# yisol/IDM-VTON

Measured on NVIDIA H100. Metric: try-on images/sec @768x1024, 30 steps, CFG 2.0, higher is better.
Workload: dtype fp16

## Files before the change

### idm-vton_b200/csrc/gemm.cu

```cuda
#include "gemm_common.cuh"
#include "host.h"
#include "wgmma.cuh"

namespace vton {

enum : int { KIND_F16 = 0, KIND_F16IN_F32OUT = 1, KIND_TF32 = 2, KIND_E4M3 = 3 };

constexpr bool f16_out(int kind) { return kind == KIND_F16 || kind == KIND_E4M3; }

template <int BN, int STAGES, bool GEGLU, int KIND>
struct SmemLayout {
  static constexpr int B_BYTES = BN * 128;
  static constexpr int STAGE_BYTES = A_BYTES + B_BYTES;
  static constexpr int STAGING_OFFSET = STAGES * STAGE_BYTES;
  static constexpr int STAGING_BYTES = f16_out(KIND) ? StagingTile<BN, GEGLU>::BYTES : 0;
  static constexpr int BAR_OFFSET = STAGING_OFFSET + STAGING_BYTES;
  static constexpr int ROWS_OFFSET = BAR_OFFSET + 256;
  static constexpr int TOTAL = ROWS_OFFSET + (f16_out(KIND) ? 2 * BM * 4 : 0) + 1024;
};

constexpr int GEMM_THREADS = 384;
constexpr int GEMM_PRODUCER_REGS = 56;
constexpr int GEMM_CONSUMER_REGS = 224;

template <int BN>
constexpr int E4M3_SUB = BN == 256 ? 64 : (BN == 192 ? 96 : BN);

template <int BN, int STAGES, bool GEGLU, bool SC, int KIND>
__global__ void __launch_bounds__(GEMM_THREADS, 1)
gemm_conv_kernel(const __grid_constant__ CUtensorMap tmA, const __grid_constant__ CUtensorMap tmB,
                 const __grid_constant__ CUtensorMap tmS0, const __grid_constant__ CUtensorMap tmS1,
                 const __grid_constant__ CUtensorMap tmBs, const GemmParams p) {
  using L = SmemLayout<BN, STAGES, GEGLU, KIND>;
  constexpr int KBK = KIND == KIND_TF32 ? 32 : (KIND == KIND_E4M3 ? 128 : 64);
  constexpr bool F16_EPI = f16_out(KIND);
  extern __shared__ uint8_t smem_raw[];
  const uint32_t smem_base = (smem_u32(smem_raw) + 1023u) & ~1023u;
  const uint32_t bar_base = smem_base + L::BAR_OFFSET;
  auto full_bar = [&](int s) { return bar_base + 8u * s; };
  auto empty_bar = [&](int s) { return bar_base + 8u * (STAGES + s); };
  const uint32_t staged_bar = bar_base + 8u * (2 * STAGES);
  const uint32_t ready_bar = bar_base + 8u * (2 * STAGES + 1);
  const uint32_t staging = smem_base + L::STAGING_OFFSET;
  auto staging_ptr = [&]() { return smem_raw + (smem_base - smem_u32(smem_raw)) + L::STAGING_OFFSET; };
  auto row_table = [&]() { return reinterpret_cast<int*>(smem_raw + (smem_base - smem_u32(smem_raw)) + L::ROWS_OFFSET); };

  const int warp = threadIdx.x >> 5;

  if (threadIdx.x == 8 * 32) {
    tma_prefetch_desc(&tmA);
    tma_prefetch_desc(&tmB);
    if (SC) {
      tma_prefetch_desc(&tmS0);
      tma_prefetch_desc(&tmS1);
      tma_prefetch_desc(&tmBs);
    }
    for (int s = 0; s < STAGES; ++s) {
      mbar_init(full_bar(s), 1);
      mbar_init(empty_bar(s), 2);
    }
    if (F16_EPI) {
      mbar_init(staged_bar, 256);
      mbar_init(ready_bar, EpilogueStore<BN, GEGLU>::THREADS);
    }
    fence_barrier_init();
  }
  pdl_wait();
  __syncthreads();
  pdl_launch_dependents();

  if (warp >= 8) {
    setmaxnreg_dec<GEMM_PRODUCER_REGS>();
    if (threadIdx.x == 8 * 32) {
      const int total_slabs = p.slabs_main + (SC ? p.slabs_sc : 0);
      uint32_t it = 0;
      for (int tile = blockIdx.x; tile < p.total_tiles; tile += gridDim.x) {
        const int n0 = (tile % p.n_tiles) * BN;
        const int m_tile = tile / p.n_tiles;
        int b0 = 0, y0 = 0, x0 = 0;
        if (p.conv) {
          x0 = (m_tile % p.tiles_x) * p.bw;
          y0 = ((m_tile / p.tiles_x) % p.tiles_y) * p.bh;
          b0 = (m_tile / (p.tiles_x * p.tiles_y)) * p.bb;
        }
        for (int s = 0; s < total_slabs; ++s, ++it) {
          const int stage = it % STAGES;
          const uint32_t phase = (it / STAGES) & 1;
          mbar_wait(empty_bar(stage), phase ^ 1);
          const uint32_t a_dst = smem_base + stage * L::STAGE_BYTES;
          const uint32_t b_dst = a_dst + A_BYTES;
          mbar_expect_tx(full_bar(stage), L::STAGE_BYTES);
          if (s < p.slabs_main) {
            if (p.conv) {
              const int tap = s / p.cin_slabs;
              const int c0 = (s - tap * p.cin_slabs) * KBK;
              const int dy = tap / 3 - 1, dx = tap % 3 - 1;
              tma_load_4d(a_dst, &tmA, full_bar(stage), c0, x0 * p.stride + dx, y0 * p.stride + dy, b0);
              tma_load_2d(b_dst, &tmB, full_bar(stage), c0, tap * p.cout + n0);
            } else {
              tma_load_2d(a_dst, &tmA, full_bar(stage), s * KBK, m_tile * BM);
              tma_load_2d(b_dst, &tmB, full_bar(stage), s * KBK, n0);
            }
          } else {
            const int ss = s - p.slabs_main;
            if (ss < p.sc_split)
              tma_load_4d(a_dst, &tmS0, full_bar(stage), ss * BK, x0, y0, b0);
            else
              tma_load_4d(a_dst, &tmS1, full_bar(stage), (ss - p.sc_split) * BK, x0, y0, b0);
            tma_load_2d(b_dst, &tmBs, full_bar(stage), ss * BK, n0);
          }
        }
      }
    } else if (F16_EPI && warp > 8) {
      EpilogueStore<BN, GEGLU>::run(p, staging, staging_ptr(), row_table(), staged_bar, ready_bar, threadIdx.x - 9 * 32);
    }
    return;
  }

  setmaxnreg_inc<GEMM_CONSUMER_REGS>();
  const int wg = warp >> 2;
  const int lane = threadIdx.x & 31;
  const int r_local = wg * 64 + ((warp & 3) << 4) + (lane >> 2);
  float acc[BN / 2];
  float acc_sc[BN / 2];
  uint32_t it = 0;
  auto release = [&](uint32_t slab) {
    if ((threadIdx.x & 127) == 0) mbar_arrive(empty_bar(slab % STAGES));
  };
  auto run_slabs = [&](float (&accr)[BN / 2], int s_begin, int s_end) {
    for (int s = s_begin; s < s_end; ++s, ++it) {
      const int stage = it % STAGES;
      mbar_wait(full_bar(stage), (it / STAGES) & 1);
      const uint32_t a_src = smem_base + stage * L::STAGE_BYTES + wg * (64 * 128);
      const uint32_t b_src = smem_base + stage * L::STAGE_BYTES + A_BYTES;
      wgmma_fence();
#pragma unroll
      for (int k = 0; k < 4; ++k) {
        const uint64_t da = make_gmma_desc_sw128(a_src + k * 32, 0, 1024);
        const uint64_t db = make_gmma_desc_sw128(b_src + k * 32, 0, 1024);
        const int scale_d = (s > s_begin || k > 0) ? 1 : 0;
        if constexpr (KIND == KIND_TF32) {
          WgmmaTF32SS<BN>::mma(accr, da, db, scale_d);
        } else {
          WgmmaF16SS<BN, 0>::mma(accr, da, db, scale_d);
        }
      }
      wgmma_commit();
      wgmma_wait<1>();
      if (s > 0) release(it - 1);
    }
  };
  auto run_slabs_promoted = [&](float (&accr)[BN / 2], int s_begin, int s_end) {
    constexpr int SUB = E4M3_SUB<BN>;
    for (int s = s_begin; s < s_end; ++s, ++it) {
      const int stage = it % STAGES;
      mbar_wait(full_bar(stage), (it / STAGES) & 1);
      const uint32_t a_src = smem_base + stage * L::STAGE_BYTES + wg * (64 * 128);
      const uint32_t b_src = smem_base + stage * L::STAGE_BYTES + A_BYTES;
#pragma unroll
      for (int sub = 0; sub < BN / SUB; ++sub) {
        float part[SUB / 2];
        wgmma_fence();
#pragma unroll
        for (int k = 0; k < 4; ++k) {
          const uint64_t da = make_gmma_desc_sw128(a_src + k * 32, 0, 1024);
          const uint64_t db = make_gmma_desc_sw128(b_src + sub * SUB * 128 + k * 32, 0, 1024);
          WgmmaE4M3SS<SUB>::mma(part, da, db, k > 0 ? 1 : 0);
        }
        wgmma_commit();
        wgmma_wait<0>();
        fence_regs(part);
#pragma unroll
        for (int j = 0; j < SUB / 2; ++j) accr[sub * (SUB / 2) + j] = s > s_begin ? accr[sub * (SUB / 2) + j] + part[j] : part[j];
      }
      release(it);
    }
  };
  for (int tile = blockIdx.x; tile < p.total_tiles; tile += gridDim.x) {
    EpilogueF16<BN, GEGLU, SC, KIND == KIND_E4M3> epi;
    if constexpr (F16_EPI) epi.begin(p, tile / p.n_tiles, tile % p.n_tiles, r_local);
    if constexpr (KIND == KIND_E4M3) {
      run_slabs_promoted(acc, 0, p.slabs_main);
    } else {
      run_slabs(acc, 0, p.slabs_main);
      if constexpr (SC) run_slabs(acc_sc, p.slabs_main, p.slabs_main + p.slabs_sc);
      wgmma_wait<0>();
      fence_regs(acc);
      if (SC) fence_regs(acc_sc);
      release(it - 1);
    }
    if constexpr (F16_EPI) {
      mbar_wait(ready_bar, ((tile - blockIdx.x) / gridDim.x) & 1);
      if (!GEGLU && p.act_gelu) epi.template stage<true, true>(p, acc, acc_sc, r_local, staging);
      else if (!GEGLU && p.rowvec) epi.template stage<false, true>(p, acc, acc_sc, r_local, staging);
      else epi.template stage<false, false>(p, acc, acc_sc, r_local, staging);
      mbar_arrive(staged_bar);
      if (tile + static_cast<int>(gridDim.x) >= p.total_tiles)
        EpilogueStore<BN, GEGLU>::help_store_last(p, tile, staging_ptr(), row_table(), staged_bar, threadIdx.x);
    } else {
      epilogue_f32<BN>(p, tile / p.n_tiles, tile % p.n_tiles, r_local, acc);
    }
  }
}

template <int BN, int STAGES, bool GEGLU, bool SC, int KIND>
static int launch_variant(const CUtensorMap& tmA, const CUtensorMap& tmB, const CUtensorMap& tmS0,
                          const CUtensorMap& tmS1, const CUtensorMap& tmBs, const GemmParams& p, cudaStream_t stream) {
  using L = SmemLayout<BN, STAGES, GEGLU, KIND>;
  static_assert(L::TOTAL <= 227 * 1024, "shared memory budget");
  auto kern = gemm_conv_kernel<BN, STAGES, GEGLU, SC, KIND>;
  static bool configured = false;
  if (!configured) {
    VTON_CUDA(cudaFuncSetAttribute(kern, cudaFuncAttributeMaxDynamicSharedMemorySize, L::TOTAL));
    configured = true;
  }
  const int grid = p.total_tiles < num_sms() ? p.total_tiles : num_sms();
  VTON_CUDA(launch_kernel(kern, dim3(grid), dim3(GEMM_THREADS), L::TOTAL, stream, tmA, tmB, tmS0, tmS1, tmBs, p));
  count_launch();
  return kOk;
}

void set_auto_v2(int) {}
void set_cluster4(int) {}

static int pick_bn(int N, int m_tiles, bool geglu, bool has_shortcut, int force_bn) {
  if (force_bn >= 2000) force_bn -= 2000;
  else if (force_bn >= 1000) force_bn -= 1000;
  auto usable = [&](int bn) {
    if (geglu && ((bn != 256 && bn != 128) || N % bn != 0)) return false;
    if (has_shortcut && bn > 128) return false;
    return true;
  };
  if (force_bn) {
    const bool known = force_bn == 64 || force_bn == 128 || force_bn == 160 || force_bn == 192 || force_bn == 256;
    return known && usable(force_bn) ? force_bn : 0;
  }
  const int sms = num_sms();
  const int cands[5] = {256, 192, 160, 128, 64};
  double best = 1e300;
  int best_bn = 0;
  for (int bn : cands) {
    if (!usable(bn)) continue;
    if (bn != 128 && N % bn != 0 && !(bn == 64 && N < 64)) continue;
    const long long tiles = static_cast<long long>(m_tiles) * cdiv(N, bn);
    const long long waves = (tiles + sms - 1) / sms;
    const double cost = static_cast<double>(waves) * (bn + 64);
    if (cost < best * 0.999) {
      best = cost;
      best_bn = bn;
    }
  }
  return best_bn ? best_bn : 128;
}

template <int KIND>
static int dispatch(int bn, bool geglu, const CUtensorMap& tmA, const CUtensorMap& tmB, const CUtensorMap& tmS0,
                    const CUtensorMap& tmS1, const CUtensorMap& tmBs, GemmParams& p, int m_tiles,
                    cudaStream_t stream) {
  p.n_tiles = cdiv(p.N, bn);
  p.total_tiles = m_tiles * p.n_tiles;
  if (geglu) {
    if (bn == 128) return launch_variant<128, 6, true, false, KIND>(tmA, tmB, tmS0, tmS1, tmBs, p, stream);
    if (bn == 256) return launch_variant<256, 4, true, false, KIND>(tmA, tmB, tmS0, tmS1, tmBs, p, stream);
    set_last_error("GEGLU epilogue supports BN 128/256 only (got %d)", bn);
    return kErrUnsupported;
  }
  if constexpr (KIND == KIND_F16) {
    if (p.slabs_sc) {
      if (bn == 64) return launch_variant<64, 8, false, true, KIND_F16>(tmA, tmB, tmS0, tmS1, tmBs, p, stream);
      if (bn == 128) return launch_variant<128, 6, false, true, KIND_F16>(tmA, tmB, tmS0, tmS1, tmBs, p, stream);
      set_last_error("shortcut epilogue supports BN 64/128 only (got %d)", bn);
      return kErrUnsupported;
    }
  }
  switch (bn) {
    case 64: return launch_variant<64, 8, false, false, KIND>(tmA, tmB, tmS0, tmS1, tmBs, p, stream);
    case 128: return launch_variant<128, 6, false, false, KIND>(tmA, tmB, tmS0, tmS1, tmBs, p, stream);
    case 160: return launch_variant<160, 5, false, false, KIND>(tmA, tmB, tmS0, tmS1, tmBs, p, stream);
    case 192: return launch_variant<192, 4, false, false, KIND>(tmA, tmB, tmS0, tmS1, tmBs, p, stream);
    case 256: return launch_variant<256, 3, false, false, KIND>(tmA, tmB, tmS0, tmS1, tmBs, p, stream);
  }
  set_last_error("unsupported BN %d", bn);
  return kErrUnsupported;
}

int gemm_f16_impl(const void* A, long long lda, const void* W, long long ldw, void* out, long long ldo, int M, int N,
                  int K, const void* bias, const void* residual, long long ldr, const void* rowvec, long long ld_rowvec,
                  int rows_per_sample, int flags, int force_bn, cudaStream_t stream) {
  const int geglu = flags & 1;
  VTON_CHECK_ARG(M > 0 && N > 0 && K > 0, "gemm: empty problem M=%d N=%d K=%d", M, N, K);
  VTON_CHECK_ARG(K % 64 == 0, "gemm: K=%d must be a multiple of 64", K);
  VTON_CHECK_ARG(N % 8 == 0 && lda % 8 == 0 && ldw % 8 == 0 && ldo % 8 == 0, "gemm: N/lda/ldw/ldo must be multiples of 8");
  VTON_CHECK_ARG(!geglu || (N % 16 == 0 && !residual && !rowvec), "gemm: bad GEGLU configuration");
  VTON_CHECK_ARG(aligned_to(out, 16) && aligned_to(bias, 16) && aligned_to(residual, 16) && aligned_to(rowvec, 16),
                 "gemm: out/bias/residual/rowvec must be 16-byte aligned");
  VTON_CHECK_ARG((!residual || ldr % 8 == 0) && (!rowvec || ld_rowvec % 8 == 0),
                 "gemm: ldr=%lld / ld_rowvec=%lld must be multiples of 8", ldr, ld_rowvec);
  const int bn = pick_bn(N, cdiv(M, BM), geglu != 0, false, force_bn);
  VTON_CHECK_ARG(bn != 0, "gemm: tile width force_bn=%d unsupported for this problem (N=%d, geglu=%d)", force_bn, N, geglu);
  VTON_CHECK_ARG(!geglu || N % bn == 0, "gemm: GEGLU needs N %% BN == 0 (N=%d, BN=%d)", N, bn);
  CUtensorMap tmA, tmB;
  {
    uint64_t dims[2] = {static_cast<uint64_t>(K), static_cast<uint64_t>(M)};
    uint64_t strides[1] = {static_cast<uint64_t>(lda) * 2};
    uint32_t box[2] = {64, 128};
    if (int e = encode_tmap_f16(&tmA, A, 2, dims, strides, box)) return e;
  }
  {
    uint64_t dims[2] = {static_cast<uint64_t>(K), static_cast<uint64_t>(N)};
    uint64_t strides[1] = {static_cast<uint64_t>(ldw) * 2};
    uint32_t box[2] = {64, static_cast<uint32_t>(bn)};
    if (int e = encode_tmap_f16(&tmB, W, 2, dims, strides, box)) return e;
  }
  GemmParams p{};
  p.out = static_cast<__half*>(out);
  p.ld_out = static_cast<int>(ldo);
  p.M = M;
  p.N = N;
  p.bias = static_cast<const __half*>(bias);
  p.residual = static_cast<const __half*>(residual);
  p.ld_res = static_cast<int>(ldr);
  p.rowvec = static_cast<const __half*>(rowvec);
  p.ld_rowvec = static_cast<int>(ld_rowvec);
  p.rows_per_sample = rows_per_sample;
  p.slabs_main = K / 64;
  p.act_gelu = (flags & 4) ? 2 : ((flags & 2) ? 1 : 0);
  return dispatch<KIND_F16>(bn, geglu != 0, tmA, tmB, tmA, tmA, tmB, p, cdiv(M, BM), stream);
}

int gemm_e4m3_impl(const void* A, long long lda, const void* a_scale, const void* W, long long ldw, const void* w_scale,
                   void* out, long long ldo, int M, int N, int K, const void* bias, const void* residual, long long ldr,
                   int flags, int force_bn, cudaStream_t stream) {
  const int geglu = flags & 1;
  VTON_CHECK_ARG(M > 0 && N > 0 && K > 0, "gemm_e4m3: empty problem M=%d N=%d K=%d", M, N, K);
  VTON_CHECK_ARG(K % 128 == 0, "gemm_e4m3: K=%d must be a multiple of 128", K);
  VTON_CHECK_ARG((flags & ~1) == 0, "gemm_e4m3: flags=%d unsupported (only GEGLU = 1)", flags);
  VTON_CHECK_ARG(A && W && out && a_scale && w_scale, "gemm_e4m3: A, W, out, a_scale and w_scale must not be null");
  VTON_CHECK_ARG(lda % 16 == 0 && ldw % 16 == 0, "gemm_e4m3: lda=%lld / ldw=%lld must be multiples of 16 bytes", lda, ldw);
  VTON_CHECK_ARG(N % 8 == 0 && ldo % 8 == 0, "gemm_e4m3: N/ldo must be multiples of 8");
  VTON_CHECK_ARG(!geglu || (N % 16 == 0 && !residual), "gemm_e4m3: bad GEGLU configuration");
  VTON_CHECK_ARG(aligned_to(A, 16) && aligned_to(W, 16) && aligned_to(out, 16) && aligned_to(bias, 16) &&
                     aligned_to(residual, 16) && aligned_to(a_scale, 4) && aligned_to(w_scale, 8),
                 "gemm_e4m3: A/W/out/bias/residual must be 16-byte aligned, a_scale 4-byte, w_scale 8-byte");
  VTON_CHECK_ARG(!residual || ldr % 8 == 0, "gemm_e4m3: ldr=%lld must be a multiple of 8", ldr);
  const int bn = pick_bn(N, cdiv(M, BM), geglu != 0, false, force_bn);
  VTON_CHECK_ARG(bn != 0, "gemm_e4m3: tile width force_bn=%d unsupported for this problem (N=%d, geglu=%d)", force_bn, N,
                 geglu);
  VTON_CHECK_ARG(!geglu || N % bn == 0, "gemm_e4m3: GEGLU needs N %% BN == 0 (N=%d, BN=%d)", N, bn);
  CUtensorMap tmA, tmB;
  {
    uint64_t dims[2] = {static_cast<uint64_t>(K), static_cast<uint64_t>(M)};
    uint64_t strides[1] = {static_cast<uint64_t>(lda)};
    uint32_t box[2] = {128, 128};
    if (int e = encode_tmap_u8(&tmA, A, 2, dims, strides, box)) return e;
  }
  {
    uint64_t dims[2] = {static_cast<uint64_t>(K), static_cast<uint64_t>(N)};
    uint64_t strides[1] = {static_cast<uint64_t>(ldw)};
    uint32_t box[2] = {128, static_cast<uint32_t>(bn)};
    if (int e = encode_tmap_u8(&tmB, W, 2, dims, strides, box)) return e;
  }
  GemmParams p{};
  p.out = static_cast<__half*>(out);
  p.ld_out = static_cast<int>(ldo);
  p.M = M;
  p.N = N;
  p.bias = static_cast<const __half*>(bias);
  p.residual = static_cast<const __half*>(residual);
  p.ld_res = static_cast<int>(ldr);
  p.slabs_main = K / 128;
  p.a_scale = static_cast<const float*>(a_scale);
  p.w_scale = static_cast<const float*>(w_scale);
  return dispatch<KIND_E4M3>(bn, geglu != 0, tmA, tmB, tmA, tmA, tmB, p, cdiv(M, BM), stream);
}

static void pick_box(int B, int H, int W, int* bw, int* bh, int* bb) {
  int w = 1;
  while (w < 128 && W % (w * 2) == 0) w *= 2;
  int h = 1;
  while (w * h < 128 && h * 2 <= H) h *= 2;
  *bw = w;
  *bh = h;
  *bb = 128 / (w * h);
  (void)B;
}

static int encode_nhwc(CUtensorMap* tm, const void* base, int B, int H, int W, int C, int ldc, int bw, int bh, int bb,
                       int pixel_step = 1) {
  uint64_t dims[4] = {static_cast<uint64_t>(C), static_cast<uint64_t>(W), static_cast<uint64_t>(H),
                      static_cast<uint64_t>(B)};
  uint64_t strides[3] = {static_cast<uint64_t>(ldc) * 2, static_cast<uint64_t>(W) * ldc * 2,
                         static_cast<uint64_t>(H) * W * ldc * 2};
  uint32_t box[4] = {64, static_cast<uint32_t>(bw * pixel_step), static_cast<uint32_t>(bh * pixel_step),
                     static_cast<uint32_t>(bb)};
  uint32_t estr[4] = {1, static_cast<uint32_t>(pixel_step), static_cast<uint32_t>(pixel_step), 1};
  return encode_tmap_f16(tm, base, 4, dims, strides, box, pixel_step > 1 ? estr : nullptr);
}

int conv3x3_impl(const void* x, long long ldx, int B, int Hin, int Win, int Cin, const void* w, int Cout, const void* bias,
                 const void* temb, long long ld_temb, const void* sc0, int C0, const void* sc1, int C1, const void* w_sc,
                 const void* bias_sc, const void* residual, long long ldr, void* out, long long ldo, int force_bn,
                 int stride, cudaStream_t stream) {
  VTON_CHECK_ARG(B > 0 && Hin > 0 && Win > 0, "conv3x3: empty input");
  VTON_CHECK_ARG(stride == 1 || stride == 2, "conv3x3: stride %d unsupported", stride);
  VTON_CHECK_ARG(stride == 1 || (!w_sc && !residual), "conv3x3: stride 2 has no shortcut / residual form");
  const int H = (Hin - 1) / stride + 1, W = (Win - 1) / stride + 1;
  VTON_CHECK_ARG(Cin % 64 == 0, "conv3x3: Cin=%d must be a multiple of 64 (pad channels)", Cin);
  VTON_CHECK_ARG(Cout % 8 == 0 && ldo % 8 == 0 && ldx % 8 == 0, "conv3x3: Cout/ldo/ldx must be multiples of 8");
  VTON_CHECK_ARG(C0 % 64 == 0 && C1 % 64 == 0, "conv3x3: shortcut source channels must be multiples of 64");
  VTON_CHECK_ARG(!(w_sc && residual), "conv3x3: shortcut conv and identity residual are exclusive");
  VTON_CHECK_ARG(aligned_to(out, 16) && aligned_to(bias, 16) && aligned_to(temb, 16) && aligned_to(bias_sc, 16) &&
                     aligned_to(residual, 16),
                 "conv3x3: out/bias/temb/bias_sc/residual must be 16-byte aligned");
  VTON_CHECK_ARG((!residual || ldr % 8 == 0) && (!temb || ld_temb % 8 == 0),
                 "conv3x3: ldr=%lld / ld_temb=%lld must be multiples of 8", ldr, ld_temb);
  int bw, bh, bb;
  pick_box(B, H, W, &bw, &bh, &bb);
  const int m_tiles_est = (W / bw) * cdiv(H, bh) * cdiv(B, bb);
  const int bn = pick_bn(Cout, m_tiles_est, false, w_sc != nullptr, force_bn);
  VTON_CHECK_ARG(bn != 0, "conv3x3: tile width force_bn=%d unsupported (a fused shortcut takes 64 or 128)", force_bn);
  CUtensorMap tmA, tmB, tmS0, tmS1, tmBs;
  VTON_CHECK_ARG(stride == 1 || (bw * 2 <= 256 && bh * 2 <= 256), "conv3x3: stride-2 box too large");
  if (int e = encode_nhwc(&tmA, x, B, Hin, Win, Cin, static_cast<int>(ldx), bw, bh, bb, stride)) return e;
  {
    uint64_t dims[2] = {static_cast<uint64_t>(Cin), static_cast<uint64_t>(9) * Cout};
    uint64_t strides[1] = {static_cast<uint64_t>(Cin) * 2};
    uint32_t box[2] = {64, static_cast<uint32_t>(bn)};
    if (int e = encode_tmap_f16(&tmB, w, 2, dims, strides, box)) return e;
  }
  tmS0 = tmA;
  tmS1 = tmA;
  tmBs = tmB;
  GemmParams p{};
  if (w_sc) {
    VTON_CHECK_ARG(sc0 && C0 > 0, "conv3x3: shortcut needs a source");
    if (int e = encode_nhwc(&tmS0, sc0, B, H, W, C0, C0, bw, bh, bb)) return e;
    if (sc1 && C1 > 0) {
      if (int e = encode_nhwc(&tmS1, sc1, B, H, W, C1, C1, bw, bh, bb)) return e;
    }
    const int Csc = C0 + (sc1 ? C1 : 0);
    uint64_t dims[2] = {static_cast<uint64_t>(Csc), static_cast<uint64_t>(Cout)};
    uint64_t strides[1] = {static_cast<uint64_t>(Csc) * 2};
    uint32_t box[2] = {64, static_cast<uint32_t>(bn)};
    if (int e = encode_tmap_f16(&tmBs, w_sc, 2, dims, strides, box)) return e;
    p.slabs_sc = Csc / 64;
    p.sc_split = C0 / 64;
  }
  p.out = static_cast<__half*>(out);
  p.ld_out = static_cast<int>(ldo);
  p.M = B * H * W;
  p.N = Cout;
  p.bias = static_cast<const __half*>(bias);
  p.bias_sc = static_cast<const __half*>(bias_sc);
  p.residual = static_cast<const __half*>(residual);
  p.ld_res = static_cast<int>(ldr);
  p.rowvec = static_cast<const __half*>(temb);
  p.ld_rowvec = static_cast<int>(ld_temb);
  p.slabs_main = 9 * (Cin / 64);
  p.conv = 1;
  p.stride = stride;
  p.H = H;
  p.W = W;
  p.B = B;
  p.bw = bw;
  p.bh = bh;
  p.bb = bb;
  p.tiles_x = W / bw;
  p.tiles_y = cdiv(H, bh);
  p.cin_slabs = Cin / 64;
  p.cout = Cout;
  const int m_tiles = p.tiles_x * p.tiles_y * cdiv(B, bb);
  return dispatch<KIND_F16>(bn, false, tmA, tmB, tmS0, tmS1, tmBs, p, m_tiles, stream);
}

int conv3x3_f32_impl(const void* x, int B, int H, int W, int Cin, const void* w, int Cout, const void* bias,
                     const void* residual, void* out, int in_fp16, cudaStream_t stream) {
  VTON_CHECK_ARG(B > 0 && H > 0 && W > 0, "conv3x3_f32: empty input");
  VTON_CHECK_ARG(Cin % 32 == 0 && Cout % 32 == 0 && Cout >= 64, "conv3x3_f32: Cin=%d / Cout=%d must be multiples of 32 (Cout >= 64)", Cin, Cout);
  VTON_CHECK_ARG(!in_fp16 || Cin % 64 == 0, "conv3x3_f32: fp16 operands need Cin=%d to be a multiple of 64", Cin);
  VTON_CHECK_ARG(x && w && out, "conv3x3_f32: null pointer");
  const int esz = in_fp16 ? 2 : 4;
  const int bk = in_fp16 ? 64 : 32;
  int bw, bh, bb;
  pick_box(B, H, W, &bw, &bh, &bb);
  VTON_CHECK_ARG(bw * bh * bb == 128 && bw >= 8, "conv3x3_f32: W=%d H=%d cannot be tiled into 128-pixel boxes", W, H);
  const int m_tiles = (W / bw) * cdiv(H, bh) * cdiv(B, bb);
  const int bn = pick_bn(Cout, m_tiles, false, false, Cout % 256 == 0 ? 256 : 128);
  CUtensorMap tmA, tmB;
  {
    uint64_t dims[4] = {static_cast<uint64_t>(Cin), static_cast<uint64_t>(W), static_cast<uint64_t>(H), static_cast<uint64_t>(B)};
    uint64_t strides[3] = {static_cast<uint64_t>(Cin) * esz, static_cast<uint64_t>(W) * Cin * esz,
                           static_cast<uint64_t>(H) * W * Cin * esz};
    uint32_t box[4] = {static_cast<uint32_t>(bk), static_cast<uint32_t>(bw), static_cast<uint32_t>(bh), static_cast<uint32_t>(bb)};
    if (int e = in_fp16 ? encode_tmap_f16(&tmA, x, 4, dims, strides, box) : encode_tmap_f32(&tmA, x, 4, dims, strides, box)) return e;
  }
  {
    uint64_t dims[2] = {static_cast<uint64_t>(Cin), static_cast<uint64_t>(9) * Cout};
    uint64_t strides[1] = {static_cast<uint64_t>(Cin) * esz};
    uint32_t box[2] = {static_cast<uint32_t>(bk), static_cast<uint32_t>(bn)};
    if (int e = in_fp16 ? encode_tmap_f16(&tmB, w, 2, dims, strides, box) : encode_tmap_f32(&tmB, w, 2, dims, strides, box)) return e;
  }
  GemmParams p{};
  p.out_f32 = static_cast<float*>(out);
  p.bias_f32 = static_cast<const float*>(bias);
  p.res_f32 = static_cast<const float*>(residual);
  p.M = B * H * W;
  p.N = Cout;
  p.slabs_main = 9 * (Cin / bk);
  p.conv = 1;
  p.stride = 1;
  p.H = H;
  p.W = W;
  p.B = B;
  p.bw = bw;
  p.bh = bh;
  p.bb = bb;
  p.tiles_x = W / bw;
  p.tiles_y = cdiv(H, bh);
  p.cin_slabs = Cin / bk;
  p.cout = Cout;
  p.n_tiles = cdiv(Cout, bn);
  p.total_tiles = m_tiles * p.n_tiles;
  if (in_fp16) {
    if (bn == 256) return launch_variant<256, 4, false, false, KIND_F16IN_F32OUT>(tmA, tmB, tmA, tmA, tmB, p, stream);
    return launch_variant<128, 6, false, false, KIND_F16IN_F32OUT>(tmA, tmB, tmA, tmA, tmB, p, stream);
  }
  if (bn == 256) return launch_variant<256, 4, false, false, KIND_TF32>(tmA, tmB, tmA, tmA, tmB, p, stream);
  return launch_variant<128, 6, false, false, KIND_TF32>(tmA, tmB, tmA, tmA, tmB, p, stream);
}

}
```

### idm-vton_b200/csrc/gemm_common.cuh

```cuda
#pragma once
#include "common.cuh"

namespace vton {

struct GemmParams {
  __half* out;
  int ld_out;
  int M, N;
  const __half* bias;
  const __half* bias_sc;
  const __half* residual;
  int ld_res;
  const __half* rowvec;
  int ld_rowvec;
  int rows_per_sample;
  int slabs_main;
  int slabs_sc;
  int sc_split;
  int conv;
  int H, W, B;
  int bw, bh, bb;
  int tiles_x, tiles_y;
  int cin_slabs;
  int cout;
  int n_tiles;
  int total_tiles;
  int act_gelu;
  int stride;
  float* out_f32;
  const float* bias_f32;
  const float* res_f32;
  const float* a_scale;
  const float* w_scale;
};

constexpr int BM = 128;
constexpr int BK = 64;
constexpr int A_BYTES = BM * BK * 2;

__device__ __forceinline__ void map_row(const GemmParams& p, int m_tile, int r_local, long long* out_row, int* sample) {
  *out_row = -1;
  if (p.conv) {
    const int tx = m_tile % p.tiles_x;
    const int ty = (m_tile / p.tiles_x) % p.tiles_y;
    const int tb = m_tile / (p.tiles_x * p.tiles_y);
    const int lx = r_local % p.bw;
    const int ly = (r_local / p.bw) % p.bh;
    const int lb = r_local / (p.bw * p.bh);
    const int b = tb * p.bb + lb, y = ty * p.bh + ly, x = tx * p.bw + lx;
    if (b < p.B && y < p.H && x < p.W) *out_row = (static_cast<long long>(b) * p.H + y) * p.W + x;
    *sample = b;
  } else {
    const int m = m_tile * BM + r_local;
    if (m < p.M) *out_row = m;
    *sample = p.rows_per_sample > 0 ? m / p.rows_per_sample : 0;
  }
}

__device__ __forceinline__ float gelu_erf_fast(float x) {
  const float ax = fabsf(x) * 0.70710678118654752f;
  const float t = __fdividef(1.0f, fmaf(0.3275911f, ax, 1.0f));
  float poly = fmaf(t, 1.061405429f, -1.453152027f);
  poly = fmaf(poly, t, 1.421413741f);
  poly = fmaf(poly, t, -0.284496736f);
  poly = fmaf(poly, t, 0.254829592f);
  poly *= t;
  float e;
  const float arg = -ax * ax * 1.4426950408889634f;
  asm("ex2.approx.ftz.f32 %0, %1;" : "=f"(e) : "f"(arg));
  const float erf_abs = fmaf(-poly, e, 1.0f);
  const float erf_v = copysignf(erf_abs, x);
  return 0.5f * x * (1.0f + erf_v);
}

__device__ __forceinline__ void quad_transpose(uint32_t (&w)[4], int q) {
  {
    const bool odd = (q & 1) != 0;
    const uint32_t s0 = __shfl_xor_sync(0xffffffffu, odd ? w[0] : w[1], 1);
    const uint32_t s1 = __shfl_xor_sync(0xffffffffu, odd ? w[2] : w[3], 1);
    if (odd) w[0] = s0, w[2] = s1;
    else w[1] = s0, w[3] = s1;
  }
  {
    const bool hi = (q & 2) != 0;
    const uint32_t s0 = __shfl_xor_sync(0xffffffffu, hi ? w[0] : w[2], 2);
    const uint32_t s1 = __shfl_xor_sync(0xffffffffu, hi ? w[1] : w[3], 2);
    if (hi) w[0] = s0, w[1] = s1;
    else w[2] = s0, w[3] = s1;
  }
}

__device__ __forceinline__ float2 ldg_h2(const __half* src) {
  return unpack_h2(__ldg(reinterpret_cast<const uint32_t*>(src)));
}

__device__ __forceinline__ void st_shared_v4(uint32_t addr, uint32_t a, uint32_t b, uint32_t c, uint32_t d) {
  asm volatile("st.shared.v4.b32 [%0], {%1, %2, %3, %4};" ::"r"(addr), "r"(a), "r"(b), "r"(c), "r"(d) : "memory");
}
__device__ __forceinline__ uint4 ld_shared_v4(uint32_t addr) {
  uint4 v;
  asm volatile("ld.shared.v4.b32 {%0, %1, %2, %3}, [%4];" : "=r"(v.x), "=r"(v.y), "=r"(v.z), "=r"(v.w) : "r"(addr) : "memory");
  return v;
}
__device__ __forceinline__ void bulk_copy_g2s(uint32_t dst, const void* src, uint32_t bytes, uint32_t bar) {
  asm volatile("cp.async.bulk.shared::cluster.global.mbarrier::complete_tx::bytes [%0], [%1], %2, [%3];"
               ::"r"(dst), "l"(reinterpret_cast<uint64_t>(src)), "r"(bytes), "r"(bar) : "memory");
}

template <int BN, bool GEGLU>
struct StagingTile {
  static constexpr int OUT_COLS = GEGLU ? BN / 2 : BN;
  static constexpr int CHUNKS_PER_ROW = OUT_COLS / 8;
  static constexpr int BYTES = BM * OUT_COLS * 2;
  __device__ static __forceinline__ uint32_t offset(int r, int chunk) {
    return static_cast<uint32_t>(r * CHUNKS_PER_ROW + chunk) * 16u;
  }
};

template <int BN, bool GEGLU, bool SC, bool SCALED = false>
struct EpilogueF16 {
  using Staging = StagingTile<BN, GEGLU>;
  static constexpr int OUT_COLS = Staging::OUT_COLS;
  static constexpr int CHUNKS = OUT_COLS / 32;
  static constexpr bool HAS_RES = !GEGLU && !SC;

  int q, n0, out_n0, out_N;
  long long out_row[2];
  int sample[2];
  uint32_t bias[BN / 8];
  uint32_t bias_sc[SC ? BN / 8 : 1];
  float a_scale[SCALED ? 2 : 1];

  __device__ __forceinline__ void begin(const GemmParams& p, int m_tile, int n_tile, int r_local) {
    q = threadIdx.x & 3;
    n0 = n_tile * BN;
    out_n0 = GEGLU ? n_tile * (BN / 2) : n0;
    out_N = GEGLU ? p.N / 2 : p.N;
#pragma unroll
    for (int h = 0; h < 2; ++h) map_row(p, m_tile, r_local + 8 * h, &out_row[h], &sample[h]);
    if constexpr (SCALED) {
#pragma unroll
      for (int h = 0; h < 2; ++h) a_scale[h] = out_row[h] >= 0 ? __ldg(p.a_scale + out_row[h]) : 0.0f;
    }
#pragma unroll
    for (int i = 0; i < BN / 8; ++i) {
      const bool ok = n0 + i * 8 < p.N;
      bias[i] = (p.bias && ok) ? __ldg(reinterpret_cast<const uint32_t*>(p.bias + n0 + i * 8 + 2 * q)) : 0u;
      if (SC) bias_sc[i] = (p.bias_sc && ok) ? __ldg(reinterpret_cast<const uint32_t*>(p.bias_sc + n0 + i * 8 + 2 * q)) : 0u;
    }
  }

  template <bool ACT, bool ROWVEC>
  __device__ __forceinline__ void stage(const GemmParams& p, const float (&acc)[BN / 2], const float (&acc_sc)[BN / 2],
                                        int r_local, uint32_t staging) {
    const __half* rowvec_row[2];
#pragma unroll
    for (int h = 0; h < 2; ++h)
      rowvec_row[h] = (ROWVEC && p.rowvec && out_row[h] >= 0)
                          ? p.rowvec + static_cast<long long>(sample[h]) * p.ld_rowvec
                          : nullptr;
#pragma unroll
    for (int c = 0; c < CHUNKS; ++c) {
      if (out_n0 + c * 32 >= out_N) break;
#pragma unroll
      for (int h = 0; h < 2; ++h) {
        uint32_t w[4];
#pragma unroll
        for (int g = 0; g < 4; ++g) {
          const int i = 4 * c + g;
          const bool col_ok = out_n0 + i * 8 < out_N;
          float v0 = acc[4 * i + 2 * h], v1 = acc[4 * i + 2 * h + 1];
          float2 w_scale[GEGLU ? 2 : 1];
          if constexpr (SCALED) {
#pragma unroll
            for (int e = 0; e < (GEGLU ? 2 : 1); ++e) {
              const int col = n0 + (i + e * (BN / 16)) * 8 + 2 * q;
              w_scale[e] = col < p.N ? __ldg(reinterpret_cast<const float2*>(p.w_scale + col)) : make_float2(0.f, 0.f);
            }
            v0 = __fmul_rn(__fmul_rn(v0, a_scale[h]), w_scale[0].x);
            v1 = __fmul_rn(__fmul_rn(v1, a_scale[h]), w_scale[0].y);
          }
          if (GEGLU) {
            float g0 = acc[4 * (i + BN / 16) + 2 * h], g1 = acc[4 * (i + BN / 16) + 2 * h + 1];
            if constexpr (SCALED) {
              g0 = __fmul_rn(__fmul_rn(g0, a_scale[h]), w_scale[GEGLU ? 1 : 0].x);
              g1 = __fmul_rn(__fmul_rn(g1, a_scale[h]), w_scale[GEGLU ? 1 : 0].y);
            }
            if (p.bias && col_ok) {
              const float2 b = unpack_h2(bias[i]), bg = unpack_h2(bias[i + BN / 16]);
              v0 += b.x, v1 += b.y, g0 += bg.x, g1 += bg.y;
            }
            v0 = round_h(v0) * round_h(gelu_erf_fast(round_h(g0)));
            v1 = round_h(v1) * round_h(gelu_erf_fast(round_h(g1)));
          } else {
            if (p.bias && col_ok) {
              const float2 b = unpack_h2(bias[i]);
              v0 += b.x, v1 += b.y;
            }
            if (ACT && p.act_gelu) {
              const float x0 = round_h(v0), x1 = round_h(v1);
              v0 = p.act_gelu == 2 ? __fdividef(x0, 1.0f + __expf(-1.702f * x0)) : gelu_erf_fast(x0);
              v1 = p.act_gelu == 2 ? __fdividef(x1, 1.0f + __expf(-1.702f * x1)) : gelu_erf_fast(x1);
            }
            if (ROWVEC && rowvec_row[h] != nullptr && col_ok) {
              const float2 t = ldg_h2(rowvec_row[h] + n0 + i * 8 + 2 * q);
              v0 = round_h(v0) + t.x, v1 = round_h(v1) + t.y;
            }
            if (SC) {
              float s0 = acc_sc[4 * i + 2 * h], s1 = acc_sc[4 * i + 2 * h + 1];
              if (p.bias_sc && col_ok) {
                const float2 b = unpack_h2(bias_sc[i]);
                s0 += b.x, s1 += b.y;
              }
              v0 = round_h(s0) + round_h(v0), v1 = round_h(s1) + round_h(v1);
            }
          }
          w[g] = pack_h2(v0, v1);
        }
        quad_transpose(w, q);
        const uint32_t slot = staging + Staging::offset(r_local + 8 * h, 4 * c + q);
        if (HAS_RES && p.residual) {
          const uint4 u = ld_shared_v4(slot);
          const uint32_t r[4] = {u.x, u.y, u.z, u.w};
#pragma unroll
          for (int j = 0; j < 4; ++j) {
            const float2 a = unpack_h2(w[j]), d = unpack_h2(r[j]);
            w[j] = pack_h2(a.x + d.x, a.y + d.y);
          }
        }
        st_shared_v4(slot, w[0], w[1], w[2], w[3]);
      }
    }
  }
};

template <int BN, bool GEGLU>
struct EpilogueStore {
  using Staging = StagingTile<BN, GEGLU>;
  static constexpr int THREADS = 96;
  static constexpr int CPR = Staging::CHUNKS_PER_ROW;
  static constexpr int UNITS = BM * CPR;

  __device__ static __forceinline__ void store(const GemmParams& p, const uint8_t* staging_ptr, const int* rows, int out_n0,
                                               int out_N, int t, int n) {
#pragma unroll 4
    for (int u = t; u < UNITS; u += n) {
      const int r = u / CPR, chunk = u % CPR;
      const int row = rows[r];
      const int col = out_n0 + chunk * 8;
      if (row >= 0 && col < out_N)
        *reinterpret_cast<uint4*>(p.out + static_cast<long long>(row) * p.ld_out + col) =
            *reinterpret_cast<const uint4*>(staging_ptr + Staging::offset(r, chunk));
    }
  }

  __device__ static __forceinline__ void help_store_last(const GemmParams& p, int tile, const uint8_t* staging_ptr,
                                                         const int* row_table, uint32_t staged_bar, int t) {
    const int j = (tile - blockIdx.x) / gridDim.x;
    mbar_wait(staged_bar, j & 1);
    store(p, staging_ptr, row_table + (j & 1) * BM, (tile % p.n_tiles) * Staging::OUT_COLS, GEGLU ? p.N / 2 : p.N,
          THREADS + t, THREADS + 256);
  }

  __device__ static __forceinline__ void run(const GemmParams& p, uint32_t staging, const uint8_t* staging_ptr,
                                             int* row_table, uint32_t staged_bar, uint32_t ready_bar, int e) {
    const int out_N = GEGLU ? p.N / 2 : p.N;
    int j = 0;
    for (int tile = blockIdx.x; tile < p.total_tiles; tile += gridDim.x, ++j) {
      const int m_tile = tile / p.n_tiles;
      const int out_n0 = (tile % p.n_tiles) * Staging::OUT_COLS;
      int* rows = row_table + (j & 1) * BM;
      for (int r = e; r < BM; r += THREADS) {
        long long out_row;
        int sample;
        map_row(p, m_tile, r, &out_row, &sample);
        rows[r] = static_cast<int>(out_row);
      }
      named_bar_sync(1, THREADS);
      if (p.residual) {
        fence_proxy_async_smem();
        const uint32_t row_bytes = (out_N - out_n0 < Staging::OUT_COLS ? out_N - out_n0 : Staging::OUT_COLS) * 2u;
        uint32_t bytes = 0;
        for (int r = e; r < BM; r += THREADS) bytes += rows[r] >= 0 ? row_bytes : 0u;
        mbar_expect_tx(ready_bar, bytes);
        for (int r = e; r < BM; r += THREADS) {
          if (rows[r] >= 0)
            bulk_copy_g2s(staging + Staging::offset(r, 0), p.residual + static_cast<long long>(rows[r]) * p.ld_res + out_n0,
                          row_bytes, ready_bar);
        }
      } else {
        mbar_arrive(ready_bar);
      }
      mbar_wait(staged_bar, j & 1);
      const bool last = tile + static_cast<int>(gridDim.x) >= p.total_tiles;
      store(p, staging_ptr, rows, out_n0, out_N, e, last ? THREADS + 256 : THREADS);
    }
  }
};

template <int BN>
__device__ __forceinline__ void epilogue_f32(const GemmParams& p, int m_tile, int n_tile, int r_local,
                                             const float (&acc)[BN / 2]) {
  const int q = threadIdx.x & 3;
  const int n0 = n_tile * BN;
  long long out_row[2];
#pragma unroll
  for (int h = 0; h < 2; ++h) {
    int sample;
    map_row(p, m_tile, r_local + 8 * h, &out_row[h], &sample);
  }
#pragma unroll
  for (int i = 0; i < BN / 8; ++i) {
    if (n0 + i * 8 >= p.N) break;
    const int ncol = n0 + i * 8 + 2 * q;
    float2 b = make_float2(0.0f, 0.0f);
    if (p.bias_f32 != nullptr) b = __ldg(reinterpret_cast<const float2*>(p.bias_f32 + ncol));
#pragma unroll
    for (int h = 0; h < 2; ++h) {
      if (out_row[h] < 0) continue;
      float2 v = make_float2(acc[4 * i + 2 * h], acc[4 * i + 2 * h + 1]);
      if (p.bias_f32 != nullptr) v.x += b.x, v.y += b.y;
      if (p.res_f32 != nullptr) {
        const float2 r = __ldg(reinterpret_cast<const float2*>(p.res_f32 + out_row[h] * p.N + ncol));
        v.x += r.x, v.y += r.y;
      }
      *reinterpret_cast<float2*>(p.out_f32 + out_row[h] * p.N + ncol) = v;
    }
  }
}

}
```

Before: 0.9371.

## Move GEGLU gating from consumer epilogue into store warps with work split

The GEGLU epilogue no longer computes gelu(gate)*hidden in the consumer warpgroups. Instead it stages the full BN-wide fp16 tile and lets the store warps apply the gating while writing out. The store work is split between the store warps and the consumer threads by a ratio based on K-slab count, coordinated through an extra ready-barrier arrival. The aim is to shorten the consumer epilogue so the next tile's MMA can start sooner. This doubles the staging buffer size, so BN=256 GEGLU drops to 3 pipeline stages. The gelu reciprocal is also switched to rcp.approx via inline asm.

```diff
diff --git a/idm-vton_b200/csrc/gemm.cu b/idm-vton_b200/csrc/gemm.cu
--- a/idm-vton_b200/csrc/gemm.cu
+++ b/idm-vton_b200/csrc/gemm.cu
@@ -13,7 +13,7 @@
   static constexpr int B_BYTES = BN * 128;
   static constexpr int STAGE_BYTES = A_BYTES + B_BYTES;
   static constexpr int STAGING_OFFSET = STAGES * STAGE_BYTES;
-  static constexpr int STAGING_BYTES = f16_out(KIND) ? StagingTile<BN, GEGLU>::BYTES : 0;
+  static constexpr int STAGING_BYTES = f16_out(KIND) ? StagingTile<BN>::BYTES : 0;
   static constexpr int BAR_OFFSET = STAGING_OFFSET + STAGING_BYTES;
   static constexpr int ROWS_OFFSET = BAR_OFFSET + 256;
   static constexpr int TOTAL = ROWS_OFFSET + (f16_out(KIND) ? 2 * BM * 4 : 0) + 1024;
@@ -61,7 +61,7 @@
     }
     if (F16_EPI) {
       mbar_init(staged_bar, 256);
-      mbar_init(ready_bar, EpilogueStore<BN, GEGLU>::THREADS);
+      mbar_init(ready_bar, EpilogueStore<BN, GEGLU>::READY_ARRIVALS);
     }
     fence_barrier_init();
   }
@@ -124,6 +124,7 @@
   float acc[BN / 2];
   float acc_sc[BN / 2];
   uint32_t it = 0;
+  if (F16_EPI && GEGLU) mbar_arrive(ready_bar);
   auto release = [&](uint32_t slab) {
     if ((threadIdx.x & 127) == 0) mbar_arrive(empty_bar(slab % STAGES));
   };
@@ -197,6 +198,8 @@
       mbar_arrive(staged_bar);
       if (tile + static_cast<int>(gridDim.x) >= p.total_tiles)
         EpilogueStore<BN, GEGLU>::help_store_last(p, tile, staging_ptr(), row_table(), staged_bar, threadIdx.x);
+      else if (GEGLU)
+        EpilogueStore<BN, GEGLU>::help_store(p, tile, staging_ptr(), row_table(), staged_bar, ready_bar, threadIdx.x);
     } else {
       epilogue_f32<BN>(p, tile / p.n_tiles, tile % p.n_tiles, r_local, acc);
     }
@@ -261,7 +264,7 @@
   p.total_tiles = m_tiles * p.n_tiles;
   if (geglu) {
     if (bn == 128) return launch_variant<128, 6, true, false, KIND>(tmA, tmB, tmS0, tmS1, tmBs, p, stream);
-    if (bn == 256) return launch_variant<256, 4, true, false, KIND>(tmA, tmB, tmS0, tmS1, tmBs, p, stream);
+    if (bn == 256) return launch_variant<256, 3, true, false, KIND>(tmA, tmB, tmS0, tmS1, tmBs, p, stream);
     set_last_error("GEGLU epilogue supports BN 128/256 only (got %d)", bn);
     return kErrUnsupported;
   }
diff --git a/idm-vton_b200/csrc/gemm_common.cuh b/idm-vton_b200/csrc/gemm_common.cuh
--- a/idm-vton_b200/csrc/gemm_common.cuh
+++ b/idm-vton_b200/csrc/gemm_common.cuh
@@ -59,7 +59,8 @@
 
 __device__ __forceinline__ float gelu_erf_fast(float x) {
   const float ax = fabsf(x) * 0.70710678118654752f;
-  const float t = __fdividef(1.0f, fmaf(0.3275911f, ax, 1.0f));
+  float t;
+  asm("rcp.approx.ftz.f32 %0, %1;" : "=f"(t) : "f"(fmaf(0.3275911f, ax, 1.0f)));
   float poly = fmaf(t, 1.061405429f, -1.453152027f);
   poly = fmaf(poly, t, 1.421413741f);
   poly = fmaf(poly, t, -0.284496736f);
@@ -107,11 +108,10 @@
                ::"r"(dst), "l"(reinterpret_cast<uint64_t>(src)), "r"(bytes), "r"(bar) : "memory");
 }
 
-template <int BN, bool GEGLU>
+template <int BN>
 struct StagingTile {
-  static constexpr int OUT_COLS = GEGLU ? BN / 2 : BN;
-  static constexpr int CHUNKS_PER_ROW = OUT_COLS / 8;
-  static constexpr int BYTES = BM * OUT_COLS * 2;
+  static constexpr int CHUNKS_PER_ROW = BN / 8;
+  static constexpr int BYTES = BM * BN * 2;
   __device__ static __forceinline__ uint32_t offset(int r, int chunk) {
     return static_cast<uint32_t>(r * CHUNKS_PER_ROW + chunk) * 16u;
   }
@@ -119,12 +119,11 @@
 
 template <int BN, bool GEGLU, bool SC, bool SCALED = false>
 struct EpilogueF16 {
-  using Staging = StagingTile<BN, GEGLU>;
-  static constexpr int OUT_COLS = Staging::OUT_COLS;
-  static constexpr int CHUNKS = OUT_COLS / 32;
+  using Staging = StagingTile<BN>;
+  static constexpr int CHUNKS = BN / 32;
   static constexpr bool HAS_RES = !GEGLU && !SC;
 
-  int q, n0, out_n0, out_N;
+  int q, n0;
   long long out_row[2];
   int sample[2];
   uint32_t bias[BN / 8];
@@ -134,8 +133,6 @@
   __device__ __forceinline__ void begin(const GemmParams& p, int m_tile, int n_tile, int r_local) {
     q = threadIdx.x & 3;
     n0 = n_tile * BN;
-    out_n0 = GEGLU ? n_tile * (BN / 2) : n0;
-    out_N = GEGLU ? p.N / 2 : p.N;
 #pragma unroll
     for (int h = 0; h < 2; ++h) map_row(p, m_tile, r_local + 8 * h, &out_row[h], &sample[h]);
     if constexpr (SCALED) {
@@ -161,59 +158,41 @@
                           : nullptr;
 #pragma unroll
     for (int c = 0; c < CHUNKS; ++c) {
-      if (out_n0 + c * 32 >= out_N) break;
+      if (n0 + c * 32 >= p.N) break;
 #pragma unroll
       for (int h = 0; h < 2; ++h) {
         uint32_t w[4];
 #pragma unroll
         for (int g = 0; g < 4; ++g) {
           const int i = 4 * c + g;
-          const bool col_ok = out_n0 + i * 8 < out_N;
+          const bool col_ok = n0 + i * 8 < p.N;
           float v0 = acc[4 * i + 2 * h], v1 = acc[4 * i + 2 * h + 1];
-          float2 w_scale[GEGLU ? 2 : 1];
           if constexpr (SCALED) {
-#pragma unroll
-            for (int e = 0; e < (GEGLU ? 2 : 1); ++e) {
-              const int col = n0 + (i + e * (BN / 16)) * 8 + 2 * q;
-              w_scale[e] = col < p.N ? __ldg(reinterpret_cast<const float2*>(p.w_scale + col)) : make_float2(0.f, 0.f);
+            const int col = n0 + i * 8 + 2 * q;
+            const float2 w_scale = col < p.N ? __ldg(reinterpret_cast<const float2*>(p.w_scale + col)) : make_float2(0.f, 0.f);
+            v0 = __fmul_rn(__fmul_rn(v0, a_scale[h]), w_scale.x);
+            v1 = __fmul_rn(__fmul_rn(v1, a_scale[h]), w_scale.y);
+          }
+          if (p.bias && col_ok) {
+            const float2 b = unpack_h2(bias[i]);
+            v0 += b.x, v1 += b.y;
+          }
+          if (ACT && p.act_gelu) {
+            const float x0 = round_h(v0), x1 = round_h(v1);
+            v0 = p.act_gelu == 2 ? __fdividef(x0, 1.0f + __expf(-1.702f * x0)) : gelu_erf_fast(x0);
+            v1 = p.act_gelu == 2 ? __fdividef(x1, 1.0f + __expf(-1.702f * x1)) : gelu_erf_fast(x1);
+          }
+          if (ROWVEC && rowvec_row[h] != nullptr && col_ok) {
+            const float2 t = ldg_h2(rowvec_row[h] + n0 + i * 8 + 2 * q);
+            v0 = round_h(v0) + t.x, v1 = round_h(v1) + t.y;
+          }
+          if (SC) {
+            float s0 = acc_sc[4 * i + 2 * h], s1 = acc_sc[4 * i + 2 * h + 1];
+            if (p.bias_sc && col_ok) {
+              const float2 b = unpack_h2(bias_sc[i]);
+              s0 += b.x, s1 += b.y;
             }
-            v0 = __fmul_rn(__fmul_rn(v0, a_scale[h]), w_scale[0].x);
-            v1 = __fmul_rn(__fmul_rn(v1, a_scale[h]), w_scale[0].y);
-          }
-          if (GEGLU) {
-            float g0 = acc[4 * (i + BN / 16) + 2 * h], g1 = acc[4 * (i + BN / 16) + 2 * h + 1];
-            if constexpr (SCALED) {
-              g0 = __fmul_rn(__fmul_rn(g0, a_scale[h]), w_scale[GEGLU ? 1 : 0].x);
-              g1 = __fmul_rn(__fmul_rn(g1, a_scale[h]), w_scale[GEGLU ? 1 : 0].y);
-            }
-            if (p.bias && col_ok) {
-              const float2 b = unpack_h2(bias[i]), bg = unpack_h2(bias[i + BN / 16]);
-              v0 += b.x, v1 += b.y, g0 += bg.x, g1 += bg.y;
-            }
-            v0 = round_h(v0) * round_h(gelu_erf_fast(round_h(g0)));
-            v1 = round_h(v1) * round_h(gelu_erf_fast(round_h(g1)));
-          } else {
-            if (p.bias && col_ok) {
-              const float2 b = unpack_h2(bias[i]);
-              v0 += b.x, v1 += b.y;
-            }
-            if (ACT && p.act_gelu) {
-              const float x0 = round_h(v0), x1 = round_h(v1);
-              v0 = p.act_gelu == 2 ? __fdividef(x0, 1.0f + __expf(-1.702f * x0)) : gelu_erf_fast(x0);
-              v1 = p.act_gelu == 2 ? __fdividef(x1, 1.0f + __expf(-1.702f * x1)) : gelu_erf_fast(x1);
-            }
-            if (ROWVEC && rowvec_row[h] != nullptr && col_ok) {
-              const float2 t = ldg_h2(rowvec_row[h] + n0 + i * 8 + 2 * q);
-              v0 = round_h(v0) + t.x, v1 = round_h(v1) + t.y;
-            }
-            if (SC) {
-              float s0 = acc_sc[4 * i + 2 * h], s1 = acc_sc[4 * i + 2 * h + 1];
-              if (p.bias_sc && col_ok) {
-                const float2 b = unpack_h2(bias_sc[i]);
-                s0 += b.x, s1 += b.y;
-              }
-              v0 = round_h(s0) + round_h(v0), v1 = round_h(s1) + round_h(v1);
-            }
+            v0 = round_h(s0) + round_h(v0), v1 = round_h(s1) + round_h(v1);
           }
           w[g] = pack_h2(v0, v1);
         }
@@ -236,21 +215,41 @@
 
 template <int BN, bool GEGLU>
 struct EpilogueStore {
-  using Staging = StagingTile<BN, GEGLU>;
+  using Staging = StagingTile<BN>;
   static constexpr int THREADS = 96;
-  static constexpr int CPR = Staging::CHUNKS_PER_ROW;
+  static constexpr int OUT_COLS = GEGLU ? BN / 2 : BN;
+  static constexpr int CPR = OUT_COLS / 8;
   static constexpr int UNITS = BM * CPR;
+  static constexpr int GEGLU_SW_SLABS = 14;
+  static constexpr int READY_ARRIVALS = THREADS + (GEGLU ? 256 : 0);
+
+  __device__ static __forceinline__ int store_warp_units(const GemmParams& p) {
+    return !GEGLU || p.slabs_main >= GEGLU_SW_SLABS ? UNITS : p.slabs_main * UNITS / GEGLU_SW_SLABS;
+  }
+
+  __device__ static __forceinline__ uint4 geglu_chunk(const uint4& h, const uint4& g) {
+    const uint32_t hw[4] = {h.x, h.y, h.z, h.w}, gw[4] = {g.x, g.y, g.z, g.w};
+    uint32_t o[4];
+#pragma unroll
+    for (int j = 0; j < 4; ++j) {
+      const float2 v = unpack_h2(hw[j]), x = unpack_h2(gw[j]);
+      o[j] = pack_h2(v.x * round_h(gelu_erf_fast(x.x)), v.y * round_h(gelu_erf_fast(x.y)));
+    }
+    return make_uint4(o[0], o[1], o[2], o[3]);
+  }
 
   __device__ static __forceinline__ void store(const GemmParams& p, const uint8_t* staging_ptr, const int* rows, int out_n0,
-                                               int out_N, int t, int n) {
-#pragma unroll 4
-    for (int u = t; u < UNITS; u += n) {
+                                               int out_N, int u, int u_end, int n) {
+#pragma unroll(GEGLU ? 1 : 4)
+    for (; u < u_end; u += n) {
       const int r = u / CPR, chunk = u % CPR;
       const int row = rows[r];
       const int col = out_n0 + chunk * 8;
-      if (row >= 0 && col < out_N)
-        *reinterpret_cast<uint4*>(p.out + static_cast<long long>(row) * p.ld_out + col) =
-            *reinterpret_cast<const uint4*>(staging_ptr + Staging::offset(r, chunk));
+      if (row >= 0 && col < out_N) {
+        uint4 v = *reinterpret_cast<const uint4*>(staging_ptr + Staging::offset(r, chunk));
+        if constexpr (GEGLU) v = geglu_chunk(v, *reinterpret_cast<const uint4*>(staging_ptr + Staging::offset(r, CPR + chunk)));
+        *reinterpret_cast<uint4*>(p.out + static_cast<long long>(row) * p.ld_out + col) = v;
+      }
     }
   }
 
@@ -258,8 +257,19 @@
                                                          const int* row_table, uint32_t staged_bar, int t) {
     const int j = (tile - blockIdx.x) / gridDim.x;
     mbar_wait(staged_bar, j & 1);
-    store(p, staging_ptr, row_table + (j & 1) * BM, (tile % p.n_tiles) * Staging::OUT_COLS, GEGLU ? p.N / 2 : p.N,
-          THREADS + t, THREADS + 256);
+    store(p, staging_ptr, row_table + (j & 1) * BM, (tile % p.n_tiles) * OUT_COLS, GEGLU ? p.N / 2 : p.N,
+          THREADS + t, UNITS, THREADS + 256);
+  }
+
+  __device__ static __forceinline__ void help_store(const GemmParams& p, int tile, const uint8_t* staging_ptr,
+                                                    const int* row_table, uint32_t staged_bar, uint32_t ready_bar, int t) {
+    const int u0 = store_warp_units(p);
+    if (u0 < UNITS) {
+      const int j = (tile - blockIdx.x) / gridDim.x;
+      mbar_wait(staged_bar, j & 1);
+      store(p, staging_ptr, row_table + (j & 1) * BM, (tile % p.n_tiles) * OUT_COLS, p.N / 2, u0 + t, UNITS, 256);
+    }
+    mbar_arrive(ready_bar);
   }
 
   __device__ static __forceinline__ void run(const GemmParams& p, uint32_t staging, const uint8_t* staging_ptr,
@@ -268,7 +278,7 @@
     int j = 0;
     for (int tile = blockIdx.x; tile < p.total_tiles; tile += gridDim.x, ++j) {
       const int m_tile = tile / p.n_tiles;
-      const int out_n0 = (tile % p.n_tiles) * Staging::OUT_COLS;
+      const int out_n0 = (tile % p.n_tiles) * OUT_COLS;
       int* rows = row_table + (j & 1) * BM;
       for (int r = e; r < BM; r += THREADS) {
         long long out_row;
@@ -279,7 +289,7 @@
       named_bar_sync(1, THREADS);
       if (p.residual) {
         fence_proxy_async_smem();
-        const uint32_t row_bytes = (out_N - out_n0 < Staging::OUT_COLS ? out_N - out_n0 : Staging::OUT_COLS) * 2u;
+        const uint32_t row_bytes = (out_N - out_n0 < OUT_COLS ? out_N - out_n0 : OUT_COLS) * 2u;
         uint32_t bytes = 0;
         for (int r = e; r < BM; r += THREADS) bytes += rows[r] >= 0 ? row_bytes : 0u;
         mbar_expect_tx(ready_bar, bytes);
@@ -293,7 +303,7 @@
       }
       mbar_wait(staged_bar, j & 1);
       const bool last = tile + static_cast<int>(gridDim.x) >= p.total_tiles;
-      store(p, staging_ptr, rows, out_n0, out_N, e, last ? THREADS + 256 : THREADS);
+      store(p, staging_ptr, rows, out_n0, out_N, e, last ? UNITS : store_warp_units(p), last ? THREADS + 256 : THREADS);
     }
   }
 };
```

Result: faster. 0.9471 (median of 6 runs) (+1.1%).
